# Dizzy-cell/HOUV

Measured on AMD Instinct MI355X. Metric: registration pairs/sec (2048-pt partial pairs), higher is better.
Workload: dtype f32; 1 GPU; HOUV solve_model, 2048x2048-pt pairs, batch 256/GPU, K=64 restarts x 200 Adam iterations + retry stages (BASELINE configs[1]); pairs_per_gpu=256, points=2048, kernel=64, iters=200, icp_refine=False, parallelism=dp1 (pair shards, one RCCL all-gather of [steps*P,12] per rank)

## Files before the change

houv_amd/csrc/capi.hip:

```cpp
#include <stdarg.h>
#include <string.h>

#include "../../include/houv_hip.h"
#include "houv_common.h"

namespace houv {

static thread_local char g_err[512] = "";

void set_error(const char* fmt, ...) {
  va_list ap;
  va_start(ap, fmt);
  vsnprintf(g_err, sizeof(g_err), fmt, ap);
  va_end(ap);
  fprintf(stderr, "[houv_hip] %s\n", g_err);
}

DebugKnobs g_debug;

namespace {

__global__ void pose_kernel(const float* __restrict__ params, int n, int angle_base, int trans_mode,
                            float* __restrict__ R, float* __restrict__ T) {
  const int i = blockIdx.x * blockDim.x + threadIdx.x;
// ... 15 lines not shown
    const size_t b = e / N;
    const float* r = R + b * 9;
    const float x = src[e * 3 + 0], y = src[e * 3 + 1], z = src[e * 3 + 2];
    moved[e * 3 + 0] = __builtin_fmaf(z, r[2], __builtin_fmaf(y, r[1], x * r[0])) + T[b * 3 + 0];
    moved[e * 3 + 1] = __builtin_fmaf(z, r[5], __builtin_fmaf(y, r[4], x * r[3])) + T[b * 3 + 1];
    moved[e * 3 + 2] = __builtin_fmaf(z, r[8], __builtin_fmaf(y, r[7], x * r[6])) + T[b * 3 + 2];
  }
}

}
}

extern "C" int houv_abi_version(void) { return HOUV_ABI_VERSION; }

extern "C" const char* houv_last_error(void) { return houv::g_err; }

extern "C" int houv_debug_set(const char* name, long long value) {
  using namespace houv;
  const struct { const char* name; std::atomic<int>* knob; long long lo, hi, step; } ints[] = {
      {"solve_predict", &g_debug.pred_mode, 0, 2, 1}, {"knn_split", &g_debug.knn_split, 0, 1, 1},
      {"attn_split", &g_debug.attn_split, 0, 1, 1},   {"gemm_split", &g_debug.gemm_split, 0, 6, 3}};
  if (name && !strcmp(name, "solve_stats")) {
    g_debug.stats = (unsigned long long)value;
    return 1;
  }
  if (name && !strcmp(name, "solve_walk_hist")) {
    g_debug.walk_hist = (unsigned long long)value;
    return 1;
  }
  if (name && !strcmp(name, "solve_cull_stats")) {
    g_debug.cull_stats = (unsigned long long)value;
    return 1;
  }
  for (const auto& k : ints)
    if (name && !strcmp(name, k.name) && value >= k.lo && value <= k.hi && value % k.step == 0) {
      *k.knob = (int)value;
      return 1;
    }
  set_error("houv_debug_set: unknown switch or value out of range: %s = %lld", name ? name : "(null)", value);
  return 0;
}

#ifndef HOUV_BUILD_ID
#define HOUV_BUILD_ID "unknown"
#endif
extern "C" const char* houv_build_id(void) { return HOUV_BUILD_ID; }

extern "C" int houv_pose_forward(const float* params, int n, int angle_base, int trans_mode, const float* src, int N,
                                 float* R, float* T, float* moved, void* stream) {
  using namespace houv;
  if (n < 0 || !params || !R || !T || angle_base < 0 || angle_base > 3 || trans_mode < 0 || trans_mode > 1) {
    set_error("houv_pose_forward: bad argument");
    return 0;
  }
  if (n == 0) return 1;
  hipStream_t s = (hipStream_t)stream;
  pose_kernel<<<(n + 255) / 256, 256, 0, s>>>(params, n, angle_base, trans_mode, R, T);
  if (src && moved && N > 0) {
    const size_t total = (size_t)n * N;
    size_t blocks = (total + 255) / 256;
    if (blocks > 16384) blocks = 16384;
    move_kernel<<<(unsigned)blocks, 256, 0, s>>>(src, R, T, total, N, moved);
  }
  return check_launch("houv_pose_forward") ? 1 : 0;
}
```

houv_amd/csrc/houv_common.h:

```cpp
#pragma once
#include <hip/hip_runtime.h>
#include <stdint.h>
#include <stdio.h>

#include <atomic>

#include "houv_math.h"

namespace houv {

constexpr int kWave = 64;
constexpr int kSub = 32;
constexpr int kTrk = 16;

void set_error(const char* fmt, ...);
struct SolveCommon;
__attribute__((visibility("hidden"))) int solve_check_args(const char* who, const SolveCommon& a, int use_views);
__attribute__((visibility("hidden"))) bool scatter_index_launch(const int* keys, int B, int N, int M, int* offsets, int* order,
                                                                hipStream_t stream);
inline bool check_launch(const char* what) {
  hipError_t e = hipGetLastError();
  if (e != hipSuccess) {
    set_error("%s: %s", what, hipGetErrorString(e));
    return false;
  }
  return true;
}

struct DebugKnobs {
  std::atomic<int> pred_mode{0};
  std::atomic<unsigned long long> stats{0ull};
  std::atomic<unsigned long long> walk_hist{0ull};
  std::atomic<unsigned long long> cull_stats{0ull};
  std::atomic<int> knn_split{1};
  std::atomic<int> attn_split{1};
  std::atomic<int> gemm_split{6};
};
extern DebugKnobs g_debug;

template <int MET>
__device__ __forceinline__ float metric_sqdist(float dx, float dy, float dz) {
  if constexpr (MET == 0) return __builtin_fmaf(dz, dz, __builtin_fmaf(dy, dy, dx * dx));
  else if constexpr (MET == 1) return __builtin_fmaf(dz, dz, dy * dy);
  else if constexpr (MET == 2) return __builtin_fmaf(dz, dz, dx * dx);
  else return __builtin_fmaf(dy, dy, dx * dx);
}

__device__ __forceinline__ float min3f(float a, float b, float c) {
  return __builtin_fminf(__builtin_fminf(a, b), c);
}

__device__ __forceinline__ float wave_sum(float v) {
#pragma unroll
  for (int o = 32; o > 0; o >>= 1) v += __shfl_xor(v, o, kWave);
  return v;
}

__device__ __forceinline__ int wave_sum_i(int v) {
#pragma unroll
  for (int o = 32; o > 0; o >>= 1) v += __shfl_xor(v, o, kWave);
  return v;
}

template <int CTRL, int ROW_MASK = 0xf, int BANK_MASK = 0xf>
__device__ __forceinline__ float dpp_f(float v) {
  return __int_as_float(__builtin_amdgcn_update_dpp(0, __float_as_int(v), CTRL, ROW_MASK, BANK_MASK, true));
// ... 63 lines not shown
```

houv_amd/csrc/houv_math.h:

```cpp
#pragma once
#include <math.h>

#if defined(__HIPCC__)
#define HOUV_HD __host__ __device__
#else
#define HOUV_HD
#endif

namespace houv {

constexpr float kPiF = 3.14159274101257324f;

enum TransMode { kTransHouv = 0, kTransSolve = 1 };

HOUV_HD inline float tsqrt(float x) { return sqrtf(x); }
HOUV_HD inline double tsqrt(double x) { return sqrt(x); }

struct Pose {
  float R[9];
  float T[3];
  float u[3], inv_vnorm, sin_t, cos_t, chat[3], inv_cnorm, sigma, a, s;
};

HOUV_HD inline void pose_forward(const float p[8], int angle_base, int trans_mode, Pose& o) {
  const float vx = p[0], vy = p[1], vz = p[2];
  const float vn = sqrtf(vx * vx + vy * vy + vz * vz);
  o.inv_vnorm = 1.0f / vn;
  o.u[0] = vx / vn; o.u[1] = vy / vn; o.u[2] = vz / vn;
  o.a = p[3];
  const float theta = sinf(p[3] * kPiF) * kPiF / 8.0f + kPiF / 8.0f + (float)angle_base * kPiF / 4.0f;
  const float st = sinf(theta), ct = cosf(theta);
  o.sin_t = st; o.cos_t = ct;
  const float ux = o.u[0], uy = o.u[1], uz = o.u[2];
  const float A[9] = {0.f, -uz, uy, uz, 0.f, -ux, -uy, ux, 0.f};
  float AA[9];
  for (int i = 0; i < 3; ++i)
    for (int j = 0; j < 3; ++j)
      AA[i * 3 + j] = A[i * 3 + 0] * A[0 * 3 + j] + A[i * 3 + 1] * A[1 * 3 + j] + A[i * 3 + 2] * A[2 * 3 + j];
  const float omc = 1.0f - ct;
  for (int i = 0; i < 9; ++i) o.R[i] = ((i % 4 == 0) ? 1.0f : 0.0f) + st * A[i] + omc * AA[i];
  o.s = p[7];
  const float sp = sinf(p[7] * kPiF);
  o.sigma = (trans_mode == kTransHouv) ? (sp * 0.125f + 0.125f) : (sp * 1.0f);
  const float cx = p[4], cy = p[5], cz = p[6];
  const float cn = sqrtf(cx * cx + cy * cy + cz * cz);
  o.inv_cnorm = 1.0f / cn;
  o.chat[0] = cx / cn; o.chat[1] = cy / cn; o.chat[2] = cz / cn;
  o.T[0] = o.chat[0] * o.sigma; o.T[1] = o.chat[1] * o.sigma; o.T[2] = o.chat[2] * o.sigma;
}

HOUV_HD inline void pose_backward(const Pose& f, int trans_mode, const float gT[3], const float M[9], float g[8]) {
  const float ux = f.u[0], uy = f.u[1], uz = f.u[2];
  const float A[9] = {0.f, -uz, uy, uz, 0.f, -ux, -uy, ux, 0.f};
  float AA[9], MAt[9], AtM[9];
  for (int i = 0; i < 3; ++i)
    for (int j = 0; j < 3; ++j) {
      AA[i * 3 + j] = A[i * 3 + 0] * A[0 * 3 + j] + A[i * 3 + 1] * A[1 * 3 + j] + A[i * 3 + 2] * A[2 * 3 + j];
      MAt[i * 3 + j] = M[i * 3 + 0] * A[j * 3 + 0] + M[i * 3 + 1] * A[j * 3 + 1] + M[i * 3 + 2] * A[j * 3 + 2];
      AtM[i * 3 + j] = A[0 * 3 + i] * M[0 * 3 + j] + A[1 * 3 + i] * M[1 * 3 + j] + A[2 * 3 + i] * M[2 * 3 + j];
    }
  float dth = 0.f;
  for (int i = 0; i < 9; ++i) dth += M[i] * (f.cos_t * A[i] + f.sin_t * AA[i]);
  g[3] = dth * cosf(f.a * kPiF) * kPiF * kPiF / 8.0f;
  float Qm[9];
  const float omc = 1.0f - f.cos_t;
  for (int i = 0; i < 9; ++i) Qm[i] = f.sin_t * M[i] + omc * (MAt[i] + AtM[i]);
  const float du0 = Qm[7] - Qm[5], du1 = Qm[2] - Qm[6], du2 = Qm[3] - Qm[1];
  const float dot_u = ux * du0 + uy * du1 + uz * du2;
  g[0] = (du0 - ux * dot_u) * f.inv_vnorm;
  g[1] = (du1 - uy * dot_u) * f.inv_vnorm;
  g[2] = (du2 - uz * dot_u) * f.inv_vnorm;
  const float dot_c = f.chat[0] * gT[0] + f.chat[1] * gT[1] + f.chat[2] * gT[2];
  g[4] = f.sigma * (gT[0] - f.chat[0] * dot_c) * f.inv_cnorm;
  g[5] = f.sigma * (gT[1] - f.chat[1] * dot_c) * f.inv_cnorm;
  g[6] = f.sigma * (gT[2] - f.chat[2] * dot_c) * f.inv_cnorm;
  const float dsig = (trans_mode == kTransHouv) ? (cosf(f.s * kPiF) * kPiF * 0.125f) : (cosf(f.s * kPiF) * kPiF);
  g[7] = dot_c * dsig;
}

struct AdamScalars {
  double step_size, bc2_sqrt;
};
HOUV_HD inline AdamScalars adam_scalars(int step, double lr, double b1, double b2) {
  const double bc1 = 1.0 - pow(b1, (double)step);
  const double bc2 = 1.0 - pow(b2, (double)step);
  return AdamScalars{lr / bc1, sqrt(bc2)};
}
template <typename T>
HOUV_HD inline void adam_step(T& p, T& m, T& v, T g, const AdamScalars& sc, double b1, double b2, double eps) {
  m = m + (g - m) * (T)(1.0 - b1);
  v = v * (T)b2 + ((T)(1.0 - b2) * g) * g;
  const T denom = tsqrt(v) / (T)sc.bc2_sqrt + (T)eps;
  p = p - (T)sc.step_size * (m / denom);
}
template <typename T>
HOUV_HD inline void adam_step(T& p, T& m, T& v, T g, int step, double lr, double b1, double b2, double eps) {
  adam_step<T>(p, m, v, g, adam_scalars(step, lr, b1, b2), b1, b2, eps);
}

constexpr int kAccN = 13;
constexpr int kAccStride = 16;

struct TailLoss {
  float score, loss;
  float cd[4][2];
  float g[8];
};

template <int NMET>
HOUV_HD inline void solve_tail_loss(const float* acc, int acc_stride, const Pose& f, int k_full, int k_view, float loss_scale,
// ... 19 lines not shown
#pragma unroll
    for (int i = 0; i < 9; ++i) Mm[i] += w * ac[4 + i];
  }
  r.score = val[0];
  r.loss = val[0] * 6.0f;
  if constexpr (NMET == 4) r.loss = r.loss + (val[1] + val[2] + val[3]);
  if (bad) {
#pragma unroll
    for (int i = 0; i < 3; ++i) gT[i] = NAN;
#pragma unroll
    for (int i = 0; i < 9; ++i) Mm[i] = NAN;
  }
  pose_backward(f, trans_mode, gT, Mm, r.g);
}

HOUV_HD inline void solve_tail_step(const float g[8], double* state, int f64_params, AdamScalars asc, double beta1, double beta2,
                                    double eps, int angle_base, int trans_mode, Pose& next) {
  if (f64_params) {
    for (int k = 0; k < 8; ++k)
      adam_step<double>(state[k], state[8 + k], state[16 + k], (double)g[k], asc, beta1, beta2, eps);
  } else {
    for (int k = 0; k < 8; ++k) {
      float pp = (float)state[k], mm = (float)state[8 + k], vv = (float)state[16 + k];
      adam_step<float>(pp, mm, vv, g[k], asc, beta1, beta2, eps);
      state[k] = pp; state[8 + k] = mm; state[16 + k] = vv;
    }
  }
  float p[8];
#pragma unroll
  for (int k = 0; k < 8; ++k) p[k] = (float)state[k];
  pose_forward(p, angle_base, trans_mode, next);
}

constexpr int kTermAnchorFloats = 20;
constexpr float kTermRel = 1e-3f;
constexpr float kTermAbs = 1e-6f;
constexpr float kTermMoveErr = 1e-6f;

template <int NMET>
HOUV_HD inline unsigned term_masks(const float* anchor, const float* R, const float* T, float radius) {
  float fr = 0.f, ft = 0.f, tn = 0.f, ta = 0.f;
#pragma unroll
  for (int i = 0; i < 9; ++i) {
    const float d = R[i] - anchor[8 + i];
    fr += d * d;
  }
#pragma unroll
  for (int i = 0; i < 3; ++i) {
    const float d = T[i] - anchor[17 + i];
    ft += d * d;
    tn += T[i] * T[i];
    ta += anchor[17 + i] * anchor[17 + i];
  }
  const float delta2 = 2.0f * (sqrtf(fr) * radius + sqrtf(ft));
  const float abs_margin = kTermAbs + kTermMoveErr * (2.0f * radius + sqrtf(tn) + sqrtf(ta));
  unsigned need = ((1u << NMET) - 1u) * 0x11u;
#pragma unroll
  for (int m = 0; m < NMET; ++m) {
    const float c0 = anchor[2 * m], c1 = anchor[2 * m + 1];
    const float slack = delta2 + kTermRel * (fabsf(c0) + fabsf(c1) + delta2) + abs_margin;
    const unsigned drop1 = (c0 + slack < c1) ? (0x10u << m) : 0u;
    const unsigned drop0 = (c1 + slack < c0) ? (1u << m) : 0u;
    need &= ~(drop0 | drop1);
  }
  return need;
}

constexpr float kTermDefectMax = 1e-3f;
constexpr float kTermDefectErr = 1e-6f;

HOUV_HD inline float term_rot_defect(const float* M) {
  float s = 0.f;
#pragma unroll
  for (int i = 0; i < 3; ++i)
#pragma unroll
    for (int j = i; j < 3; ++j) {
      const float g = M[i] * M[j] + M[3 + i] * M[3 + j] + M[6 + i] * M[6 + j] - ((i == j) ? 1.0f : 0.0f);
      s += ((i == j) ? 1.0f : 2.0f) * g * g;
    }
  return sqrtf(s) + kTermDefectErr;
}

HOUV_HD inline void term_travel(const float* Rz, const float* Tz, const float* R, const float* T, float def_now, float radius,
                                float& d, float& tz) {
  float fr = 0.f, ft = 0.f, ta = 0.f;
#pragma unroll
  for (int i = 0; i < 9; ++i) {
    const float e = R[i] - Rz[i];
    fr += e * e;
  }
#pragma unroll
  for (int i = 0; i < 3; ++i) {
    const float e = T[i] - Tz[i];
    ft += e * e;
    ta += Tz[i] * Tz[i];
  }
  const float fro = sqrtf(fr), defect = def_now + term_rot_defect(Rz);
  const float tight = fro * 0.70710683f + 2.0f * defect;
  const bool ok = (fr <= 2.0f) & (defect <= kTermDefectMax) & (tight < fro);
  d = (ok ? tight : fro) * radius + sqrtf(ft);
  tz = sqrtf(ta);
}

template <int NMET>
HOUV_HD inline unsigned term_anchor_masks(const float* cd, const float* fresh, const float* stale, int stride,
                                          unsigned stale_bits, const float* R, const float* T, float radius_in) {
  const float radius = fabsf(radius_in);
  const float def_now = term_rot_defect(R);
  const float tn = sqrtf(T[0] * T[0] + T[1] * T[1] + T[2] * T[2]);
  float d_f, t_f;
  term_travel(fresh, fresh + 9, R, T, def_now, radius, d_f, t_f);
  unsigned need = ((1u << NMET) - 1u) * 0x11u;
#pragma unroll
  for (int m = 0; m < NMET; ++m) {
    float Rs[9], Ts[3], d_s, t_s;
#pragma unroll
    for (int i = 0; i < 9; ++i) Rs[i] = stale[(m * 12 + i) * stride];
#pragma unroll
    for (int i = 0; i < 3; ++i) Ts[i] = stale[(m * 12 + 9 + i) * stride];
    term_travel(Rs, Ts, R, T, def_now, radius, d_s, t_s);
    const bool s0 = (stale_bits >> m) & 1u, s1 = (stale_bits >> (4 + m)) & 1u;
    const float d0 = s0 ? d_s : d_f, d1 = s1 ? d_s : d_f;
    const float t0 = s0 ? t_s : t_f, t1 = s1 ? t_s : t_f;
    const float c0 = cd[2 * m], c1 = cd[2 * m + 1];
    const float dd = d0 + d1;
    const float slack = dd + kTermRel * (fabsf(c0) + fabsf(c1) + dd) + kTermAbs +
                        kTermMoveErr * (2.0f * radius + tn + 0.5f * (t0 + t1));
    const unsigned drop1 = (c0 + slack < c1) ? (0x10u << m) : 0u;
    const unsigned drop0 = (c1 + slack < c0) ? (1u << m) : 0u;
    need &= ~(drop0 | drop1);
  }
  return need;
}

constexpr int kWalkSets[] = {6, 11, 12, 13, 15};
constexpr int kNumWalkSets = (int)(sizeof(kWalkSets) / sizeof(kWalkSets[0]));
constexpr int walk_step_cost(unsigned mset) {
  const int k0 = (int)(mset & 1u), k1 = (int)((mset >> 1) & 1u), k2 = (int)((mset >> 2) & 1u), k3 = (int)((mset >> 3) & 1u);
  return 16 * (2 * (k0 + k1 + k2 + ((k0 | k3) ? 1 : 0)) + 2 * k1 + (k0 + k1 + k2 + k3)) + 5 * (k0 + k1 + k2 + k3);
}
constexpr bool walk_instantiated(unsigned mset) {
  for (int i = 0; i < kNumWalkSets; ++i)
    if ((unsigned)kWalkSets[i] == mset) return true;
  return false;
}
constexpr unsigned walk_variant(unsigned need) {
  unsigned best = 15u;
  for (int i = 0; i < kNumWalkSets; ++i) {
    const unsigned s = (unsigned)kWalkSets[i];
    if ((s & need) == need && walk_step_cost(s) < walk_step_cost(best)) best = s;
  }
  return best;
}
static_assert(walk_instantiated(15u) && walk_variant(15u) == 15u && walk_step_cost(15u) == 16 * 14 + 20, "today's code is a variant");
constexpr unsigned long long walk_variant_table() {
  unsigned long long t = 0ull;
  for (unsigned n = 0; n < 16u; ++n) t |= (unsigned long long)walk_variant(n) << (4 * n);
  return t;
}

HOUV_HD inline float box_med3(float a, float b, float c) {
#if defined(__HIP_DEVICE_COMPILE__)
  return __builtin_amdgcn_fmed3f(a, b, c);
#else
  if (a != a || b != b || c != c) return fminf(fminf(a, b), c);
// ... 125 lines not shown
```

houv_amd/csrc/solve.hip:

```cpp
#include <stddef.h>
#include <stdlib.h>

#include "../../include/houv_hip.h"
#include "houv_common.h"
#include "houv_solve.h"

namespace houv {
namespace {

struct SolveArgs : SolveCommon {
  short* nn_ws;
  int ws_valid;
  int ws_stride;
  int pred_mode;
  unsigned long long* stats;
  unsigned long long* walk_hist;
  unsigned long long* cull_stats;
};

constexpr int kRescanBatch = 4;
constexpr int kRefresh = 4;
constexpr int kTermMaxAge = 0;

struct Smem {
  float4* tgt;
  float4* mov;
  double* state;
  double* adam;
  float* pose;
  float* acc;
  float* red;
  unsigned* hist;
  int* ctl;
  float4* tbox;
  float4* mbox;
  SortedStage st;
  float* anchor;
};
constexpr int kAnchorFloats = kTermAnchorFloats + 4;
constexpr int kTermAges = 8;
constexpr int kStalePose = 4;


__host__ __device__ inline int pad_unit(int prune) { return prune == 3 ? 2 * kSub : kSub; }

__host__ __device__ inline size_t smem_bytes(int N, int M, int block, int prune, int q) {
  const int pu = pad_unit(prune);
  int npad = (N + pu - 1) / pu * pu, mpad = (M + pu - 1) / pu * pu;
  if (prune) npad = mpad = (npad > mpad ? npad : mpad);
  const int nw = block / 64;
  const size_t nq = (size_t)block * q;
  return (size_t)(npad + mpad) * 16 + 28 * 8 + kPoseFloats * 4 + 8 * kAccStride * 4 + (size_t)2 * nw * kRedStride * 4 +
         kHistSets * kHistBins * 4 + (8 + nw) * 4 + 64 + (prune ? 2 * 128 * 16 + nq * 2 + 132 * 4 + kAnchorFloats * 4 : 0);
}

__device__ inline Smem carve(unsigned char* base, int N, int M, int block, int nq, int pu) {
  int npad = (N + pu - 1) / pu * pu, mpad = (M + pu - 1) / pu * pu;
  if (nq) npad = mpad = (npad > mpad ? npad : mpad);
  const int nw = block / 64;
  Smem s;
  s.tgt = reinterpret_cast<float4*>(base);
  s.mov = s.tgt + mpad;
  s.state = reinterpret_cast<double*>(s.mov + npad);
  s.adam = s.state + 24;
  s.pose = reinterpret_cast<float*>(s.adam + 4);
  s.acc = s.pose + kPoseFloats;
  s.red = s.acc + 8 * kAccStride;
  s.hist = reinterpret_cast<unsigned*>(s.red + 2 * nw * kRedStride);
  s.ctl = reinterpret_cast<int*>(s.hist + kHistSets * kHistBins);
  const size_t box_off = ((size_t)(reinterpret_cast<unsigned char*>(s.ctl + 8 + nw) - base) + 15) & ~(size_t)15;
  s.tbox = reinterpret_cast<float4*>(base + box_off);
  s.mbox = s.tbox + 128;
  s.st.hist = reinterpret_cast<int*>(s.mbox + 128);
  s.st.order = reinterpret_cast<unsigned short*>(s.st.hist + 132);
// ... 293 lines not shown
  if (tid == kAdamTid) {
    const int step = a.steps_done + 1;
    const AdamScalars asc = adam_scalars(step, a.lr, a.beta1, a.beta2);
    sm.adam[(step & 1) * 2 + 0] = asc.step_size;
    sm.adam[(step & 1) * 2 + 1] = asc.bc2_sqrt;
  }
  if constexpr (PRUNE) {
    float r2 = 0.f;
#pragma unroll
    for (int k = 0; k < Q; ++k) {
      float x, y, z;
      load_src_point<BLOCK>(src, k, N, x, y, z);
      const float v = __builtin_fmaf(z, z, __builtin_fmaf(y, y, x * x));
      r2 = (v <= r2) ? r2 : ((v < INFINITY) ? v : INFINITY);
    }
#pragma unroll
    for (int o = 1; o < 64; o <<= 1) r2 = fmaxf(r2, __shfl_xor(r2, o, 64));
    if ((tid & 63) == 0) sm.red[tid >> 6] = r2;
    if (tid == 0) {
      sm.ctl[0] = (int)(((1u << NMET) - 1u) * 0x11u);
      reinterpret_cast<unsigned*>(sm.anchor)[kTermAges] = 0u;
    }
  }
  __syncthreads();
  if constexpr (PRUNE) {
    if (tid == 0) {
      float r2 = 0.f;
      for (int w = 0; w < BLOCK / 64; ++w) r2 = fmaxf(r2, sm.red[w]);
      sm.anchor[kTermAnchorFloats] = sqrtf(r2) * 1.000001f;
    }
  }

  unsigned long long clk0 = 0ull, rt0 = 0ull;
  if (a.stats) {
    clk0 = __builtin_amdgcn_s_memtime();
    rt0 = __builtin_amdgcn_s_memrealtime();
  }
  constexpr int NW = BLOCK / 64;
  constexpr unsigned kAllMet = (1u << NMET) - 1u;
  unsigned pred_a = kAllMet;
  auto red_row = [&](int dir) { return sm.red + ((size_t)dir * NW + (tid_x() >> 6)) * kRedStride; };
#pragma unroll 1
  for (int it = 0; it < a.n_iters; ++it) {
    if (a.pred_mode == 1) pred_a = 0u;
    const bool allgrad = a.pred_mode == 2 || ((PRUNE != 0) && (((a.steps_done + it) % kRefresh) == 0 || (a.ws_valid == 0 && it == 0)));
    unsigned need_a = kAllMet, need_b = kAllMet;
    if constexpr (PRUNE != 0) {
      const unsigned w = (unsigned)__builtin_amdgcn_readfirstlane(*reinterpret_cast<const int*>(fresh_lds(reinterpret_cast<const float*>(sm.ctl))));
      need_b = w & kAllMet;
      need_a = (w >> 4) & kAllMet;
    }
    const unsigned grad_a = (allgrad ? kAllMet : (pred_a | ~need_b)) & need_a;
    {
      float sx[Q], sy[Q], sz[Q], mx[Q], my[Q], mz[Q];
      float R[9], T[3];
      load_rt(fresh_lds(sm.pose), R, T);
#pragma unroll
      for (int k = 0; k < Q; ++k) {
        const int i = pt_index<BLOCK>(k);
        const bool ok = i < N;
        load_src_point<BLOCK>(src, k, N, sx[k], sy[k], sz[k]);
        move_point(R, T, sx[k], sy[k], sz[k], mx[k], my[k], mz[k]);
        if (ok) sm.mov[i] = make_float4(mx[k], my[k], mz[k], 0.f);
      }
      __syncthreads();
      bool pruned_now = false;
      float best[Q][NMET];
// ... 51 lines not shown
        }
        unsigned sel[NMET];
        select_all<BLOCK, Q, NMET>(sm, best, M, a.k_full, a.k_view, need_b, hrot, sel);
        park_sqrt_sums<BLOCK, Q, NMET>(best, sel, need_b, red_row(0));
        grad_b = pick_winners();
        park_grad_sums<BLOCK, Q, NMET, 0, PRUNE != 0>(sm, sm.mov, tx, ty, tz, best, btile, sel, grad_b, M, tx, ty, tz, red_row(0), ws,
                                                     ws_b);
      } else {
        pick_winners();
      }
      const unsigned miss = pick_a & ~grad_a & kAllMet;
      if (miss) {
        if (miss & 1u) repair_direction_a<BLOCK, Q, 0>(sm, src, N, mpad, a.k_full, hrot, red_row(1));
        if constexpr (NMET == 4) {
          if (miss & 2u) repair_direction_a<BLOCK, Q, 1>(sm, src, N, mpad, a.k_view, hrot, red_row(1));
          if (miss & 4u) repair_direction_a<BLOCK, Q, 2>(sm, src, N, mpad, a.k_view, hrot, red_row(1));
          if (miss & 8u) repair_direction_a<BLOCK, Q, 3>(sm, src, N, mpad, a.k_view, hrot, red_row(1));
        }
      }
      __syncthreads();
      final_sums<BLOCK, NMET>(sm, 0, false, grad_b, kAllMet);
      if (miss) final_sums<BLOCK, NMET>(sm, 1, false, miss, kAllMet);
    }
    pred_a = pick_a;
    static_assert(NMET * kAccN <= 64, "final_sums runs on the scalar tail's wave");
    __builtin_amdgcn_wave_barrier();

    if (kAdamTid != 0 && tid == kAdamTid && it + 1 < a.n_iters) {
      const int step = a.steps_done + it + 2;
      const AdamScalars asc = adam_scalars(step, fresh(a.lr), fresh(a.beta1), fresh(a.beta2));
      sm.adam[(step & 1) * 2 + 0] = asc.step_size;
      sm.adam[(step & 1) * 2 + 1] = asc.bc2_sqrt;
    }
    if (tid == 0) {
      const int k_full = fresh(a.k_full), k_view = fresh(a.k_view);
      const float loss_scale = fresh(a.loss_scale);
      const double lr = fresh(a.lr), beta1 = fresh(a.beta1), beta2 = fresh(a.beta2), eps = fresh(a.eps);
      const int angle_base = fresh(a.angle_base), trans_mode = fresh(a.trans_mode);
      Pose f;
      load_pose(f, sm.pose);
      TailLoss r;
      solve_tail_loss<NMET>(sm.acc, kAccStride, f, k_full, k_view, loss_scale, trans_mode, r);
      if (it == a.n_iters - 1)
        store_outputs(a.out_score, a.out_loss, a.out_R, a.out_T, a.out_grad, a.out_cd, inst, f, r);
      if constexpr (PRUNE != 0) {
#pragma unroll
        for (int m = 0; m < NMET; ++m) {
          if ((need_b >> m) & 1u) sm.anchor[2 * m] = r.cd[m][0];
          if ((need_a >> m) & 1u) sm.anchor[2 * m + 1] = r.cd[m][1];
        }
      }
      const int step = a.steps_done + it + 1;
      const AdamScalars asc{sm.adam[(step & 1) * 2 + 0], sm.adam[(step & 1) * 2 + 1]};
      solve_tail_step(r.g, sm.state, a.f64_params, asc, beta1, beta2, eps, angle_base, trans_mode, f);
      if constexpr (PRUNE != 0) {
        unsigned next = kAllMet | (kAllMet << 4), ages = 0u;
        const bool all_next = fresh(a.pred_mode) == 2 || it + 2 >= a.n_iters;
        if (!all_next) {
          const unsigned have = need_b | (need_a << 4);
          float* stale = reinterpret_cast<float*>(sm.tbox) + 3;
          next = term_anchor_masks<NMET>(sm.anchor, sm.pose, stale, kStalePose, ~have & 0xffu, f.R, f.T,
                                         sm.anchor[kTermAnchorFloats]);
          const unsigned old_ages = reinterpret_cast<const unsigned*>(sm.anchor)[kTermAges];
#pragma unroll
          for (int m = 0; m < NMET; ++m) {
            unsigned age = (old_ages >> (8 * m)) & 0xffu;
            age = (((next >> m) & (next >> (4 + m)) & 1u) != 0u) ? 0u : age + 1u;
            if (kTermMaxAge > 0 && age > (unsigned)kTermMaxAge) {
              next |= 0x11u << m;
              age = 0u;
            }
            if (age > 0xffu) age = 0xffu;
            ages |= age << (8 * m);
            if (((have & ~next) >> m) & 0x11u) {
#pragma unroll
              for (int i = 0; i < 12; ++i) stale[(m * 12 + i) * kStalePose] = sm.pose[i];
            }
          }
        }
        reinterpret_cast<unsigned*>(sm.anchor)[kTermAges] = ages;
        sm.ctl[0] = (int)next;
        if (a.stats) {
          atomicAdd(&a.stats[6], (unsigned long long)(__popc(need_a) + __popc(need_b)));
          atomicAdd(&a.stats[7], (unsigned long long)(2 * NMET));
        }
      }
      store_pose(sm.pose, f);
      if (kAdamTid == 0 && it + 1 < a.n_iters) {
        const AdamScalars nxt = adam_scalars(step + 1, lr, beta1, beta2);
        sm.adam[((step + 1) & 1) * 2 + 0] = nxt.step_size;
        sm.adam[((step + 1) & 1) * 2 + 1] = nxt.bc2_sqrt;
      }
    }
    __syncthreads();
  }
  if (tid_x() < 24) a.state[(size_t)inst * 24 + tid_x()] = sm.state[tid_x()];
  if (a.stats) {
    const unsigned long long dc = __builtin_amdgcn_s_memtime() - clk0, dr = __builtin_amdgcn_s_memrealtime() - rt0;
    if (tid == 0) {
      atomicAdd(&a.stats[4], dc);
      atomicAdd(&a.stats[5], dr);
    }
  }
}

template <int BLOCK, int Q, int PRUNE>
int launch(const SolveArgs& a, int use_views, hipStream_t s) {
  const size_t bytes = smem_bytes(a.N, a.M, BLOCK, PRUNE, Q);
  const int grid = a.P * a.K;
  hipError_t e;
  if (use_views) {
    e = hipFuncSetAttribute((const void*)solve_kernel<BLOCK, Q, 4, PRUNE>, hipFuncAttributeMaxDynamicSharedMemorySize, (int)bytes);
    if (e != hipSuccess) { set_error("houv_solve_iterate: cannot reserve %zu B of LDS: %s", bytes, hipGetErrorString(e)); return 0; }
    solve_kernel<BLOCK, Q, 4, PRUNE><<<grid, BLOCK, bytes, s>>>(a);
  } else {
    e = hipFuncSetAttribute((const void*)solve_kernel<BLOCK, Q, 1, PRUNE>, hipFuncAttributeMaxDynamicSharedMemorySize, (int)bytes);
    if (e != hipSuccess) { set_error("houv_solve_iterate: cannot reserve %zu B of LDS: %s", bytes, hipGetErrorString(e)); return 0; }
    solve_kernel<BLOCK, Q, 1, PRUNE><<<grid, BLOCK, bytes, s>>>(a);
  }
  return check_launch("houv_solve_iterate") ? 1 : 0;
}

}
}

extern "C" int houv_solve_variant(int N, int M, int pruned, int* block, int* points_per_lane, int* prune_mode) {
  using namespace houv;
  const int mx = N > M ? N : M;
  if (N <= 0 || M <= 0) {
    set_error("houv_solve_variant: bad cloud sizes N=%d M=%d", N, M);
    return 0;
  }
  if (mx > 4096) {
    set_error("houv_solve_iterate: clouds larger than 4096 points do not fit in 160 KiB of LDS (N=%d M=%d)", N, M);
    return 0;
// ... 35 lines not shown
  const int P = a.P, N = a.N, M = a.M;
  if (P < 0 || N <= 0 || M <= 0 || a.K <= 0 || a.n_iters <= 0 || a.steps_done < 0 || a.angle_base < 0 || a.angle_base > 3 ||
      a.trans_mode < 0 || a.trans_mode > 1) {
    set_error("%s: bad argument P=%d N=%d M=%d K=%d n_iters=%d steps_done=%d base=%d trans_mode=%d", who, P, N, M, a.K,
              a.n_iters, a.steps_done, a.angle_base, a.trans_mode);
    return 0;
  }
  if (P == 0) return 1;
  if (!a.src || !a.tgt || !a.state) {
    set_error("%s: null pointer", who);
    return 0;
  }
  const int kv = use_views ? a.k_view : 1;
  if (a.k_full < 1 || a.k_full > N || a.k_full > M || kv < 1 || kv > N || kv > M) {
    set_error("%s: top-k size out of range (k_full=%d k_view=%d N=%d M=%d)", who, a.k_full, a.k_view, N, M);
    return 0;
  }
  if ((long long)P * a.K > 0x7fffffffLL) {
    set_error("%s: too many hypotheses", who);
    return 0;
  }
  return 2;
}

static int solve_dispatch(const houv::SolveCommon& c, int use_views, short* nn_ws, int ws_valid, int ws_stride, bool prune,
                          void* stream, const char* who) {
  using namespace houv;
  const int ok = solve_check_args(who, c, use_views);
  if (ok < 2) return ok;
  const int N = c.N, M = c.M;
  SolveArgs a{c, nn_ws, ws_valid, ws_stride, g_debug.pred_mode.load(),
              reinterpret_cast<unsigned long long*>(g_debug.stats.load()),
              reinterpret_cast<unsigned long long*>(g_debug.walk_hist.load()),
              reinterpret_cast<unsigned long long*>(g_debug.cull_stats.load())};
  hipStream_t s = (hipStream_t)stream;
  const int mx = N > M ? N : M;
  int block = 0, q = 0, mode = 0;
  if (!houv_solve_variant(N, M, prune ? 1 : 0, &block, &q, &mode)) return 0;
  if (prune && (!nn_ws || ws_stride < mx || (ws_stride & 7))) {
    set_error("%s: pruned mode needs a workspace of 16 x ws_stride int16 per hypothesis, ws_stride >= max(N,M) and a multiple of 8", who);
    return 0;
  }
  if (prune && ((uintptr_t)nn_ws & 15)) {
    set_error("%s: the pruned-mode workspace must be 16-byte aligned", who);
    return 0;
  }
  if (prune && ws_valid < 0) {
    a.ws_valid = 0;
    mode = 0;
  }
  if (mode == 0) a.nn_ws = nullptr;
#define HOUV_GO(B_, Q_)                                                          \
  if (block == B_ && q == Q_) {                                                  \
    if (mode == 2) return launch<B_, Q_, ((B_ >= 256 && Q_ >= 2) ? 2 : 0)>(a, use_views, s);    \
    return launch<B_, Q_, 0>(a, use_views, s);                                   \
  }
  if (mx <= 2048) {
    HOUV_GO(64, 1) HOUV_GO(128, 1) HOUV_GO(256, 1) HOUV_GO(256, 2) HOUV_GO(256, 3) HOUV_GO(256, 4)
    HOUV_GO(512, 3) HOUV_GO(512, 4)
  } else {
    if (block == 1024 && q == 3) return mode == 3 ? launch<1024, 3, 3>(a, use_views, s) : launch<1024, 3, 0>(a, use_views, s);
    if (block == 1024 && q == 4) return mode == 3 ? launch<1024, 4, 3>(a, use_views, s) : launch<1024, 4, 0>(a, use_views, s);
  }
#undef HOUV_GO
  set_error("%s: no kernel variant <%d,%d>", who, block, q);
  return 0;
}
// ... 22 lines not shown
```

Baseline: 217.0 pairs/s.

## Spread per-iteration solve tail across one wavefront instead of a single thread

The per-iteration serial tail (loss reduction, pose backward, Adam update, pose forward, termination anchor checks) previously ran on thread 0 alone. It now runs across the first wave's 64 lanes. Lanes split the gradient accumulation, the two trig cosines, the 8 Adam parameters and the two pose halves, and exchange values through LDS scratch with wave barriers. Stale-anchor rotation defects and norms are cached so they are not recomputed each step, and a tail-timing stats hook is added. The aim is to shorten the serial critical path between block-wide barriers, at the cost of extra wave-level synchronisation and more code complexity.

After: 218.9 pairs/s, median of 6. Within noise of the previous version (+0.9%).

```diff
diff --git a/houv_amd/csrc/capi.hip b/houv_amd/csrc/capi.hip
--- a/houv_amd/csrc/capi.hip
+++ b/houv_amd/csrc/capi.hip
@@ -71,6 +71,10 @@
     g_debug.cull_stats = (unsigned long long)value;
     return 1;
   }
+  if (name && !strcmp(name, "solve_tail_stats")) {
+    g_debug.tail_stats = (unsigned long long)value;
+    return 1;
+  }
   for (const auto& k : ints)
     if (name && !strcmp(name, k.name) && value >= k.lo && value <= k.hi && value % k.step == 0) {
       *k.knob = (int)value;
diff --git a/houv_amd/csrc/houv_common.h b/houv_amd/csrc/houv_common.h
--- a/houv_amd/csrc/houv_common.h
+++ b/houv_amd/csrc/houv_common.h
@@ -32,6 +32,7 @@
   std::atomic<unsigned long long> stats{0ull};
   std::atomic<unsigned long long> walk_hist{0ull};
   std::atomic<unsigned long long> cull_stats{0ull};
+  std::atomic<unsigned long long> tail_stats{0ull};
   std::atomic<int> knn_split{1};
   std::atomic<int> attn_split{1};
   std::atomic<int> gemm_split{6};
diff --git a/houv_amd/csrc/houv_math.h b/houv_amd/csrc/houv_math.h
--- a/houv_amd/csrc/houv_math.h
+++ b/houv_amd/csrc/houv_math.h
@@ -22,13 +22,25 @@
   float u[3], inv_vnorm, sin_t, cos_t, chat[3], inv_cnorm, sigma, a, s;
 };
 
-HOUV_HD inline void pose_forward(const float p[8], int angle_base, int trans_mode, Pose& o) {
-  const float vx = p[0], vy = p[1], vz = p[2];
-  const float vn = sqrtf(vx * vx + vy * vy + vz * vz);
-  o.inv_vnorm = 1.0f / vn;
-  o.u[0] = vx / vn; o.u[1] = vy / vn; o.u[2] = vz / vn;
+struct PoseHalf {
+  float unit[3], inv_norm, sine;
+};
+constexpr int kPoseHalfFloats = 5;
+HOUV_HD inline PoseHalf pose_forward_half(float x, float y, float z, float w) {
+  PoseHalf h;
+  const float n = sqrtf(x * x + y * y + z * z);
+  h.inv_norm = 1.0f / n;
+  h.unit[0] = x / n; h.unit[1] = y / n; h.unit[2] = z / n;
+  h.sine = sinf(w * kPiF);
+  return h;
+}
+
+HOUV_HD inline void pose_forward_halves(const float p[8], const PoseHalf& rot, const PoseHalf& tra, int angle_base, int trans_mode,
+                                        Pose& o) {
+  o.inv_vnorm = rot.inv_norm;
+  o.u[0] = rot.unit[0]; o.u[1] = rot.unit[1]; o.u[2] = rot.unit[2];
   o.a = p[3];
-  const float theta = sinf(p[3] * kPiF) * kPiF / 8.0f + kPiF / 8.0f + (float)angle_base * kPiF / 4.0f;
+  const float theta = rot.sine * kPiF / 8.0f + kPiF / 8.0f + (float)angle_base * kPiF / 4.0f;
   const float st = sinf(theta), ct = cosf(theta);
   o.sin_t = st; o.cos_t = ct;
   const float ux = o.u[0], uy = o.u[1], uz = o.u[2];
@@ -40,16 +52,20 @@
   const float omc = 1.0f - ct;
   for (int i = 0; i < 9; ++i) o.R[i] = ((i % 4 == 0) ? 1.0f : 0.0f) + st * A[i] + omc * AA[i];
   o.s = p[7];
-  const float sp = sinf(p[7] * kPiF);
+  const float sp = tra.sine;
   o.sigma = (trans_mode == kTransHouv) ? (sp * 0.125f + 0.125f) : (sp * 1.0f);
-  const float cx = p[4], cy = p[5], cz = p[6];
-  const float cn = sqrtf(cx * cx + cy * cy + cz * cz);
-  o.inv_cnorm = 1.0f / cn;
-  o.chat[0] = cx / cn; o.chat[1] = cy / cn; o.chat[2] = cz / cn;
+  o.inv_cnorm = tra.inv_norm;
+  o.chat[0] = tra.unit[0]; o.chat[1] = tra.unit[1]; o.chat[2] = tra.unit[2];
   o.T[0] = o.chat[0] * o.sigma; o.T[1] = o.chat[1] * o.sigma; o.T[2] = o.chat[2] * o.sigma;
 }
 
-HOUV_HD inline void pose_backward(const Pose& f, int trans_mode, const float gT[3], const float M[9], float g[8]) {
+HOUV_HD inline void pose_forward(const float p[8], int angle_base, int trans_mode, Pose& o) {
+  pose_forward_halves(p, pose_forward_half(p[0], p[1], p[2], p[3]), pose_forward_half(p[4], p[5], p[6], p[7]), angle_base, trans_mode, o);
+}
+
+HOUV_HD inline float pose_backward_cosine(float w) { return cosf(w * kPiF); }
+HOUV_HD inline void pose_backward_cosines(const Pose& f, int trans_mode, const float gT[3], const float M[9], float cos_a, float cos_s,
+                                          float g[8]) {
   const float ux = f.u[0], uy = f.u[1], uz = f.u[2];
   const float A[9] = {0.f, -uz, uy, uz, 0.f, -ux, -uy, ux, 0.f};
   float AA[9], MAt[9], AtM[9];
@@ -61,7 +77,7 @@
     }
   float dth = 0.f;
   for (int i = 0; i < 9; ++i) dth += M[i] * (f.cos_t * A[i] + f.sin_t * AA[i]);
-  g[3] = dth * cosf(f.a * kPiF) * kPiF * kPiF / 8.0f;
+  g[3] = dth * cos_a * kPiF * kPiF / 8.0f;
   float Qm[9];
   const float omc = 1.0f - f.cos_t;
   for (int i = 0; i < 9; ++i) Qm[i] = f.sin_t * M[i] + omc * (MAt[i] + AtM[i]);
@@ -74,8 +90,11 @@
   g[4] = f.sigma * (gT[0] - f.chat[0] * dot_c) * f.inv_cnorm;
   g[5] = f.sigma * (gT[1] - f.chat[1] * dot_c) * f.inv_cnorm;
   g[6] = f.sigma * (gT[2] - f.chat[2] * dot_c) * f.inv_cnorm;
-  const float dsig = (trans_mode == kTransHouv) ? (cosf(f.s * kPiF) * kPiF * 0.125f) : (cosf(f.s * kPiF) * kPiF);
+  const float dsig = (trans_mode == kTransHouv) ? (cos_s * kPiF * 0.125f) : (cos_s * kPiF);
   g[7] = dot_c * dsig;
+}
+HOUV_HD inline void pose_backward(const Pose& f, int trans_mode, const float gT[3], const float M[9], float g[8]) {
+  pose_backward_cosines(f, trans_mode, gT, M, pose_backward_cosine(f.a), pose_backward_cosine(f.s), g);
 }
 
 struct AdamScalars {
@@ -161,6 +180,82 @@
   pose_forward(p, angle_base, trans_mode, next);
 }
 
+constexpr int kTailXch = 24;
+constexpr int kTailXchGrad = 16;
+
+template <int NMET>
+HOUV_HD inline void solve_tail_loss_sums(int lane, const float* acc, int acc_stride, float a_or_s, int k_full, int k_view,
+                                         float loss_scale, TailLoss& r, float* xch) {
+  float val[NMET];
+  const int j = lane < 12 ? lane : 11;
+  float a = 0.f;
+  bool bad = false;
+#pragma unroll
+  for (int m = 0; m < 4; ++m) r.cd[m][0] = r.cd[m][1] = 0.f;
+#pragma unroll
+  for (int m = 0; m < NMET; ++m) {
+    const float kk = (float)((m == 0) ? k_full : k_view);
+    r.cd[m][0] = acc[(m * 2 + 0) * acc_stride] / kk;
+    r.cd[m][1] = acc[(m * 2 + 1) * acc_stride] / kk;
+    const int pick = (r.cd[m][0] <= r.cd[m][1]) ? 0 : 1;
+    val[m] = r.cd[m][pick];
+    if (r.cd[m][0] != r.cd[m][0] || r.cd[m][1] != r.cd[m][1]) { val[m] = NAN; bad = true; }
+    const float w = ((m == 0) ? 6.0f : 1.0f) * loss_scale / kk;
+    a += w * acc[(m * 2 + pick) * acc_stride + 1 + j];
+  }
+  r.score = val[0];
+  r.loss = val[0] * 6.0f;
+  if constexpr (NMET == 4) r.loss = r.loss + (val[1] + val[2] + val[3]);
+  if (bad) a = NAN;
+  if (lane < 12) xch[lane] = a;
+  const float c = pose_backward_cosine(a_or_s);
+  if (lane < 2) xch[12 + lane] = c;
+}
+
+HOUV_HD inline void solve_tail_loss_grad(int lane, const Pose& f, int trans_mode, float* xch, TailLoss& r) {
+  float gT[3], Mm[9];
+#pragma unroll
+  for (int i = 0; i < 3; ++i) gT[i] = xch[i];
+#pragma unroll
+  for (int i = 0; i < 9; ++i) Mm[i] = xch[3 + i];
+  pose_backward_cosines(f, trans_mode, gT, Mm, xch[12], xch[13], r.g);
+  if (lane == 0) {
+#pragma unroll
+    for (int k = 0; k < 8; ++k) xch[kTailXchGrad + k] = r.g[k];
+  }
+}
+
+HOUV_HD inline void solve_tail_adam(int lane, const float* xch, double* state, int f64_params, AdamScalars asc, double beta1,
+                                    double beta2, double eps) {
+  if (lane >= 8) return;
+  const float gk = xch[kTailXchGrad + lane];
+  if (f64_params) {
+    adam_step<double>(state[lane], state[8 + lane], state[16 + lane], (double)gk, asc, beta1, beta2, eps);
+  } else {
+    float pp = (float)state[lane], mm = (float)state[8 + lane], vv = (float)state[16 + lane];
+    adam_step<float>(pp, mm, vv, gk, asc, beta1, beta2, eps);
+    state[lane] = pp; state[8 + lane] = mm; state[16 + lane] = vv;
+  }
+}
+
+HOUV_HD inline void solve_tail_halves(int lane, const double* state, float* xch) {
+  const double* s = state + (lane & 1) * 4;
+  const PoseHalf h = pose_forward_half((float)s[0], (float)s[1], (float)s[2], (float)s[3]);
+  if (lane < 2) {
+    float* x = xch + lane * kPoseHalfFloats;
+    x[0] = h.unit[0]; x[1] = h.unit[1]; x[2] = h.unit[2]; x[3] = h.inv_norm; x[4] = h.sine;
+  }
+}
+
+HOUV_HD inline void solve_tail_pose(const double* state, const float* xch, int angle_base, int trans_mode, Pose& next) {
+  float p[8];
+#pragma unroll
+  for (int k = 0; k < 8; ++k) p[k] = (float)state[k];
+  const float* x = xch + kPoseHalfFloats;
+  const PoseHalf rot{{xch[0], xch[1], xch[2]}, xch[3], xch[4]}, tra{{x[0], x[1], x[2]}, x[3], x[4]};
+  pose_forward_halves(p, rot, tra, angle_base, trans_mode, next);
+}
+
 constexpr int kTermAnchorFloats = 20;
 constexpr float kTermRel = 1e-3f;
 constexpr float kTermAbs = 1e-6f;
@@ -210,25 +305,38 @@
   return sqrtf(s) + kTermDefectErr;
 }
 
+HOUV_HD inline void term_record_consts(const float* Rz, const float* Tz, float& def_z, float& tz) {
+  float ta = 0.f;
+#pragma unroll
+  for (int i = 0; i < 3; ++i) ta += Tz[i] * Tz[i];
+  def_z = term_rot_defect(Rz);
+  tz = sqrtf(ta);
+}
+
+HOUV_HD inline float term_travel_cached(const float* Rz, const float* Tz, int stride, float def_z, const float* R, const float* T,
+                                        float def_now, float radius) {
+  float fr = 0.f, ft = 0.f;
+#pragma unroll
+  for (int i = 0; i < 9; ++i) {
+    const float e = R[i] - Rz[i * stride];
+    fr += e * e;
+  }
+#pragma unroll
+  for (int i = 0; i < 3; ++i) {
+    const float e = T[i] - Tz[i * stride];
+    ft += e * e;
+  }
+  const float fro = sqrtf(fr), defect = def_now + def_z;
+  const float tight = fro * 0.70710683f + 2.0f * defect;
+  const bool ok = (fr <= 2.0f) & (defect <= kTermDefectMax) & (tight < fro);
+  return (ok ? tight : fro) * radius + sqrtf(ft);
+}
+
 HOUV_HD inline void term_travel(const float* Rz, const float* Tz, const float* R, const float* T, float def_now, float radius,
                                 float& d, float& tz) {
-  float fr = 0.f, ft = 0.f, ta = 0.f;
-#pragma unroll
-  for (int i = 0; i < 9; ++i) {
-    const float e = R[i] - Rz[i];
-    fr += e * e;
-  }
-#pragma unroll
-  for (int i = 0; i < 3; ++i) {
-    const float e = T[i] - Tz[i];
-    ft += e * e;
-    ta += Tz[i] * Tz[i];
-  }
-  const float fro = sqrtf(fr), defect = def_now + term_rot_defect(Rz);
-  const float tight = fro * 0.70710683f + 2.0f * defect;
-  const bool ok = (fr <= 2.0f) & (defect <= kTermDefectMax) & (tight < fro);
-  d = (ok ? tight : fro) * radius + sqrtf(ft);
-  tz = sqrtf(ta);
+  float def_z;
+  term_record_consts(Rz, Tz, def_z, tz);
+  d = term_travel_cached(Rz, Tz, 1, def_z, R, T, def_now, radius);
 }
 
 template <int NMET>
@@ -260,6 +368,31 @@
     need &= ~(drop0 | drop1);
   }
   return need;
+}
+
+template <int NMET>
+HOUV_HD inline unsigned term_anchor_drops(int lane, const float* cd, const float* fresh, const float* stale,
+                                          const float* stale_consts, int stride, unsigned stale_bits, const float* R, const float* T,
+                                          float radius_in, float& def_fresh, float& t_fresh) {
+  const float radius = fabsf(radius_in);
+  const float def_now = term_rot_defect(R);
+  const float tn = sqrtf(T[0] * T[0] + T[1] * T[1] + T[2] * T[2]);
+  term_record_consts(fresh, fresh + 9, def_fresh, t_fresh);
+  const float d_f = term_travel_cached(fresh, fresh + 9, 1, def_fresh, R, T, def_now, radius), t_f = t_fresh;
+  const int m = lane < NMET ? lane : NMET - 1;
+  const float d_s = term_travel_cached(stale + m * 12 * stride, stale + (m * 12 + 9) * stride, stride, stale_consts[2 * m * stride],
+                                       R, T, def_now, radius);
+  const float t_s = stale_consts[(2 * m + 1) * stride];
+  const bool s0 = (stale_bits >> m) & 1u, s1 = (stale_bits >> (4 + m)) & 1u;
+  const float d0 = s0 ? d_s : d_f, d1 = s1 ? d_s : d_f;
+  const float t0 = s0 ? t_s : t_f, t1 = s1 ? t_s : t_f;
+  const float c0 = cd[2 * m], c1 = cd[2 * m + 1];
+  const float dd = d0 + d1;
+  const float slack = dd + kTermRel * (fabsf(c0) + fabsf(c1) + dd) + kTermAbs +
+                      kTermMoveErr * (2.0f * radius + tn + 0.5f * (t0 + t1));
+  const unsigned drop1 = (c0 + slack < c1) ? (0x10u << m) : 0u;
+  const unsigned drop0 = (c1 + slack < c0) ? (1u << m) : 0u;
+  return lane < NMET ? (drop0 | drop1) : 0u;
 }
 
 constexpr int kWalkSets[] = {6, 11, 12, 13, 15};
diff --git a/houv_amd/csrc/solve.hip b/houv_amd/csrc/solve.hip
--- a/houv_amd/csrc/solve.hip
+++ b/houv_amd/csrc/solve.hip
@@ -16,6 +16,7 @@
   unsigned long long* stats;
   unsigned long long* walk_hist;
   unsigned long long* cull_stats;
+  unsigned long long* tail_stats;
 };
 
 constexpr int kRescanBatch = 4;
@@ -40,6 +41,14 @@
 constexpr int kAnchorFloats = kTermAnchorFloats + 4;
 constexpr int kTermAges = 8;
 constexpr int kStalePose = 4;
+constexpr int kStaleConsts = 48;
+static_assert(kStaleConsts + 8 <= 128, "sm.tbox has 128 entries");
+
+__device__ __forceinline__ void tail_phase() {
+  __builtin_amdgcn_fence(__ATOMIC_RELEASE, "wavefront");
+  __builtin_amdgcn_wave_barrier();
+  __builtin_amdgcn_fence(__ATOMIC_ACQUIRE, "wavefront");
+}
 
 
 __host__ __device__ inline int pad_unit(int prune) { return prune == 3 ? 2 * kSub : kSub; }
@@ -399,7 +408,7 @@
   }
 
   unsigned long long clk0 = 0ull, rt0 = 0ull;
-  if (a.stats) {
+  if (a.stats || a.tail_stats) {
     clk0 = __builtin_amdgcn_s_memtime();
     rt0 = __builtin_amdgcn_s_memrealtime();
   }
@@ -517,75 +526,105 @@
       sm.adam[(step & 1) * 2 + 0] = asc.step_size;
       sm.adam[(step & 1) * 2 + 1] = asc.bc2_sqrt;
     }
-    if (tid == 0) {
+    if (tid < 64) {
+      const int lane = tid_x();
+      unsigned long long* const tail_stats = fresh(a.tail_stats);
+      const unsigned long long tail0 = tail_stats ? __builtin_amdgcn_s_memtime() : 0ull;
       const int k_full = fresh(a.k_full), k_view = fresh(a.k_view);
       const float loss_scale = fresh(a.loss_scale);
       const double lr = fresh(a.lr), beta1 = fresh(a.beta1), beta2 = fresh(a.beta2), eps = fresh(a.eps);
       const int angle_base = fresh(a.angle_base), trans_mode = fresh(a.trans_mode);
+      float* const xch = sm.red;
+      static_assert(2 * kRedStride >= kTailXch, "the exchange array fits in the reduction scratch of one wave");
       Pose f;
       load_pose(f, sm.pose);
       TailLoss r;
-      solve_tail_loss<NMET>(sm.acc, kAccStride, f, k_full, k_view, loss_scale, trans_mode, r);
-      if (it == a.n_iters - 1)
-        store_outputs(a.out_score, a.out_loss, a.out_R, a.out_T, a.out_grad, a.out_cd, inst, f, r);
-      if constexpr (PRUNE != 0) {
-#pragma unroll
-        for (int m = 0; m < NMET; ++m) {
-          if ((need_b >> m) & 1u) sm.anchor[2 * m] = r.cd[m][0];
-          if ((need_a >> m) & 1u) sm.anchor[2 * m + 1] = r.cd[m][1];
+      static_assert(offsetof(Pose, s) == offsetof(Pose, a) + 4, "an odd lane reads f.s one float behind f.a");
+      solve_tail_loss_sums<NMET>(lane, sm.acc, kAccStride, sm.pose[offsetof(Pose, a) / 4 + (lane & 1)], k_full, k_view, loss_scale, r, xch);
+      tail_phase();
+      solve_tail_loss_grad(lane, f, trans_mode, xch, r);
+      if (lane == 0) {
+        if (it == a.n_iters - 1)
+          store_outputs(a.out_score, a.out_loss, a.out_R, a.out_T, a.out_grad, a.out_cd, inst, f, r);
+        if constexpr (PRUNE != 0) {
+#pragma unroll
+          for (int m = 0; m < NMET; ++m) {
+            if ((need_b >> m) & 1u) sm.anchor[2 * m] = r.cd[m][0];
+            if ((need_a >> m) & 1u) sm.anchor[2 * m + 1] = r.cd[m][1];
+          }
         }
       }
       const int step = a.steps_done + it + 1;
       const AdamScalars asc{sm.adam[(step & 1) * 2 + 0], sm.adam[(step & 1) * 2 + 1]};
-      solve_tail_step(r.g, sm.state, a.f64_params, asc, beta1, beta2, eps, angle_base, trans_mode, f);
+      tail_phase();
+      solve_tail_adam(lane, xch, sm.state, a.f64_params, asc, beta1, beta2, eps);
+      tail_phase();
+      solve_tail_halves(lane, sm.state, xch);
+      tail_phase();
+      solve_tail_pose(sm.state, xch, angle_base, trans_mode, f);
       if constexpr (PRUNE != 0) {
         unsigned next = kAllMet | (kAllMet << 4), ages = 0u;
         const bool all_next = fresh(a.pred_mode) == 2 || it + 2 >= a.n_iters;
         if (!all_next) {
           const unsigned have = need_b | (need_a << 4);
           float* stale = reinterpret_cast<float*>(sm.tbox) + 3;
-          next = term_anchor_masks<NMET>(sm.anchor, sm.pose, stale, kStalePose, ~have & 0xffu, f.R, f.T,
-                                         sm.anchor[kTermAnchorFloats]);
-          const unsigned old_ages = reinterpret_cast<const unsigned*>(sm.anchor)[kTermAges];
-#pragma unroll
-          for (int m = 0; m < NMET; ++m) {
-            unsigned age = (old_ages >> (8 * m)) & 0xffu;
-            age = (((next >> m) & (next >> (4 + m)) & 1u) != 0u) ? 0u : age + 1u;
-            if (kTermMaxAge > 0 && age > (unsigned)kTermMaxAge) {
-              next |= 0x11u << m;
-              age = 0u;
-            }
-            if (age > 0xffu) age = 0xffu;
-            ages |= age << (8 * m);
-            if (((have & ~next) >> m) & 0x11u) {
-#pragma unroll
-              for (int i = 0; i < 12; ++i) stale[(m * 12 + i) * kStalePose] = sm.pose[i];
+          float def_fresh, t_fresh;
+          const unsigned drop = term_anchor_drops<NMET>(lane, sm.anchor, sm.pose, stale, stale + kStaleConsts * kStalePose, kStalePose,
+                                                        ~have & 0xffu, f.R, f.T, sm.anchor[kTermAnchorFloats], def_fresh, t_fresh);
+          const unsigned drop_b = (unsigned)__ballot((drop & kAllMet) != 0u) & kAllMet;
+          const unsigned drop_a = (unsigned)__ballot((drop >> 4) != 0u) & kAllMet;
+          next &= ~(drop_b | (drop_a << 4));
+          tail_phase();
+          if (lane == 0) {
+            const unsigned old_ages = reinterpret_cast<const unsigned*>(sm.anchor)[kTermAges];
+#pragma unroll
+            for (int m = 0; m < NMET; ++m) {
+              unsigned age = (old_ages >> (8 * m)) & 0xffu;
+              age = (((next >> m) & (next >> (4 + m)) & 1u) != 0u) ? 0u : age + 1u;
+              if (kTermMaxAge > 0 && age > (unsigned)kTermMaxAge) {
+                next |= 0x11u << m;
+                age = 0u;
+              }
+              if (age > 0xffu) age = 0xffu;
+              ages |= age << (8 * m);
+              if (((have & ~next) >> m) & 0x11u) {
+#pragma unroll
+                for (int i = 0; i < 12; ++i) stale[(m * 12 + i) * kStalePose] = sm.pose[i];
+                stale[(kStaleConsts + 2 * m) * kStalePose] = def_fresh;
+                stale[(kStaleConsts + 2 * m + 1) * kStalePose] = t_fresh;
+              }
             }
           }
         }
-        reinterpret_cast<unsigned*>(sm.anchor)[kTermAges] = ages;
-        sm.ctl[0] = (int)next;
-        if (a.stats) {
-          atomicAdd(&a.stats[6], (unsigned long long)(__popc(need_a) + __popc(need_b)));
-          atomicAdd(&a.stats[7], (unsigned long long)(2 * NMET));
+        if (lane == 0) {
+          reinterpret_cast<unsigned*>(sm.anchor)[kTermAges] = ages;
+          sm.ctl[0] = (int)next;
+          if (a.stats) {
+            atomicAdd(&a.stats[6], (unsigned long long)(__popc(need_a) + __popc(need_b)));
+            atomicAdd(&a.stats[7], (unsigned long long)(2 * NMET));
+          }
         }
       }
-      store_pose(sm.pose, f);
-      if (kAdamTid == 0 && it + 1 < a.n_iters) {
-        const AdamScalars nxt = adam_scalars(step + 1, lr, beta1, beta2);
-        sm.adam[((step + 1) & 1) * 2 + 0] = nxt.step_size;
-        sm.adam[((step + 1) & 1) * 2 + 1] = nxt.bc2_sqrt;
+      if (lane == 0) {
+        store_pose(sm.pose, f);
+        if (kAdamTid == 0 && it + 1 < a.n_iters) {
+          const AdamScalars nxt = adam_scalars(step + 1, lr, beta1, beta2);
+          sm.adam[((step + 1) & 1) * 2 + 0] = nxt.step_size;
+          sm.adam[((step + 1) & 1) * 2 + 1] = nxt.bc2_sqrt;
+        }
+        if (tail_stats) atomicAdd(&tail_stats[0], __builtin_amdgcn_s_memtime() - tail0);
       }
     }
     __syncthreads();
   }
   if (tid_x() < 24) a.state[(size_t)inst * 24 + tid_x()] = sm.state[tid_x()];
-  if (a.stats) {
+  if (a.stats || a.tail_stats) {
     const unsigned long long dc = __builtin_amdgcn_s_memtime() - clk0, dr = __builtin_amdgcn_s_memrealtime() - rt0;
-    if (tid == 0) {
+    if (tid == 0 && a.stats) {
       atomicAdd(&a.stats[4], dc);
       atomicAdd(&a.stats[5], dr);
     }
+    if (tid == 0 && a.tail_stats) atomicAdd(&a.tail_stats[1], dc);
   }
 }
 
@@ -687,7 +726,8 @@
   SolveArgs a{c, nn_ws, ws_valid, ws_stride, g_debug.pred_mode.load(),
               reinterpret_cast<unsigned long long*>(g_debug.stats.load()),
               reinterpret_cast<unsigned long long*>(g_debug.walk_hist.load()),
-              reinterpret_cast<unsigned long long*>(g_debug.cull_stats.load())};
+              reinterpret_cast<unsigned long long*>(g_debug.cull_stats.load()),
+              reinterpret_cast<unsigned long long*>(g_debug.tail_stats.load())};
   hipStream_t s = (hipStream_t)stream;
   const int mx = N > M ? N : M;
   int block = 0, q = 0, mode = 0;
```
